# mwhoffman/pygp

Measured on AMD Instinct MI355X. Metric: ExactGP log-lik+grad evals/sec at N=16384 D=8 SE-ARD fp64, higher is better.
Workload: dtype f64; 1 GPU; ExactGP SE-ARD fp64 loglik+grad, N=16384 D=8 (metric config); batched-theta path: 6 independent thetas per GPU per step through gpx_loglik_batch, X/y resident in HBM; safe_mode=False, safe_mode_switches=0, launch=one process, C ABI only (no torch)

## Files before the change

### pygp_amd/csrc/chol.hip

```cpp

#include "gpx_internal.h"

#define LB GPX_TILE

#include <algorithm>
#include <vector>

__global__ __launch_bounds__(256) void copy_block_kernel(const double *__restrict__ src,
                                                         double *__restrict__ dst, int ld,
                                                         int rows, int cols, long long stride)
{
    src += (long long)blockIdx.z * stride;
    dst += (long long)blockIdx.z * stride;
    const int c2 = blockIdx.x * 256 + threadIdx.x;
    if (2 * c2 >= cols) return;
    for (int r = blockIdx.y; r < rows; r += gridDim.y)
        reinterpret_cast<double2 *>(dst + (size_t)r * ld)[c2] =
            reinterpret_cast<const double2 *>(src + (size_t)r * ld)[c2];
}

static int copy_block(hipStream_t s, const double *src, double *dst, int ld, int rows,
                      int cols, int batch = 1, long long stride = 0)
{
    dim3 grid((cols / 2 + 255) / 256, rows < 1024 ? rows : 1024, batch);
// ... 415 lines not shown
    hipEvent_t *G = w.events + 2 * GPX_MAX_BLOCKS;
    hipEvent_t *TD = w.events + 3 * GPX_MAX_BLOCKS;
    bool lead = false;
    if (ahead) {
        GPX_EV(hipEventRecord(D[0], s));
        const bool wide0 = nb > 1 && wide_ok(w, bl.len(0), bl.len(1), 1);
        lead = w.lead && w.lead_rows >= (wide0 ? bl.off(2) : bl.len(0));
        GPX_EV(hipStreamWaitEvent(crit, lead ? w.lead : D[0], 0));
        GPX_EV(hipStreamWaitEvent(bulk, D[0], 0));
        if (aux != bulk) GPX_EV(hipStreamWaitEvent(aux, D[0], 0));
    }
    for (int k = 0; k < nb; ++k) {
        const int ok = bl.off(k), nk = bl.len(k);
        if (ahead && k > 0) GPX_EV(hipStreamWaitEvent(crit, D[k], 0));
        const bool wide = k + 1 < nb && wide_ok(w, nk, bl.len(k + 1), 1);
        if (wide)
            GPX_TRY(gpx_panel(crit, w, ok, nk, bl.len(k + 1), w.gate_total[0], w.gate_total[1]));
        else
            GPX_TRY(potrf_rec(crit, w, ok, nk, true));
        if (ahead) {
            GPX_EV(hipEventRecord(F[k], crit));
            GPX_EV(hipStreamWaitEvent(bulk, F[k], 0));
            if (lead && k == 0) GPX_EV(hipStreamWaitEvent(crit, D[0], 0));
        }
        if (fast && k + 1 < nb) {
            const int o1 = bl.off(k + 1), n1 = bl.len(k + 1), rest = w.np - o1;
            const size_t okk = (size_t)ok * ld + ok, ok1 = (size_t)ok * ld + o1;
            const size_t o11 = (size_t)o1 * ld + o1;
            if (!wide) {
                if (k >= 1) GPX_EV(hipStreamWaitEvent(crit, G[k - 1], 0));
                {
                    GemmArgs g = mk(w.W + okk, ld, w.Kinv + ok1, ld, w.A + ok1, ld, nk, n1, nk,
                                    1.0, 0.0, GEMM_KHI_M);
                    g.order = gpx_env().ord_r12;
                    GPX_TRY(gpx_gemm(crit, 1, 0, g));
                }
                if (k >= 1) GPX_EV(hipStreamWaitEvent(crit, TD[k - 1], 0));
                GPX_TRY(syrk_upper(crit, w.A + ok1, ld, w.A + o11, ld, n1, nk, w.Kinv + o11));
            }
            GPX_EV(hipEventRecord(D[k + 1], crit));
            if (rest > n1) {
                GemmArgs g = mk(w.W + okk, ld, w.Kinv + ok1 + n1, ld, w.A + ok1 + n1, ld, nk,
                                rest - n1, nk, 1.0, 0.0, GEMM_KHI_M);
                g.order = gpx_env().ord_r12;
                GPX_TRY(gpx_gemm(bulk, 1, 0, g));
            }
            GPX_EV(hipStreamWaitEvent(bulk, D[k + 1], 0));
            if (k + 2 < nb) {
                const int o2 = bl.off(k + 2), n2 = bl.len(k + 2), rest2 = w.np - o2;
                const size_t ok2 = (size_t)ok * ld + o2, o12 = (size_t)o1 * ld + o2,
                             o22 = (size_t)o2 * ld + o2;
                {
                    GemmArgs g = mk(w.A + ok1, ld, w.A + ok2, ld, w.Kinv + o12, ld, n1, rest2,
                                    nk, -1.0, 1.0, 0);
                    GPX_TRY(gpx_gemm(bulk, 1, 0, g));
                }
                GPX_TRY(gate_bump(bulk, w, 0));
                GPX_EV(hipEventRecord(G[k], bulk));
                GPX_TRY(syrk_upper(bulk, w.A + ok2, ld, w.A + o22, ld, n2, nk, w.Kinv + o22));
                GPX_TRY(gate_bump(bulk, w, 1));
                GPX_EV(hipEventRecord(TD[k], bulk));
                if (k + 3 < nb) {
                    const int o3 = bl.off(k + 3), rest3 = w.np - o3;
                    const size_t ok3 = (size_t)ok * ld + o3, o23 = (size_t)o2 * ld + o3,
                                 o33 = (size_t)o3 * ld + o3;
                    GemmArgs g = mk(w.A + ok2, ld, w.A + ok3, ld, w.Kinv + o23, ld, n2, rest3, nk,
                                    -1.0, 1.0, 0);
                    GPX_TRY(gpx_gemm(bulk, 1, 0, g));
                    GPX_TRY(syrk_upper(bulk, w.A + ok3, ld, w.A + o33, ld, rest3, nk,
                                       w.Kinv + o33));
                }
            }
        } else if (k + 1 < nb) {
            const int o1 = bl.off(k + 1), n1 = bl.len(k + 1), rest = w.np - o1;
            const size_t okk = (size_t)ok * ld + ok, ok1 = (size_t)ok * ld + o1;
            const int skip = wide ? n1 : 0;
            if (rest > skip) {
                GemmArgs g = mk(w.W + okk, ld, w.Kinv + ok1 + skip, ld, w.A + ok1 + skip, ld, nk,
                                rest - skip, nk, 1.0, 0.0, GEMM_KHI_M);
                g.order = gpx_env().ord_r12;
                GPX_TRY(gpx_gemm(bulk, 1, 0, g));
            }
            const size_t o11 = (size_t)o1 * ld + o1;
            if (!wide)
                GPX_TRY(syrk_upper(bulk, w.A + ok1, ld, w.A + o11, ld, n1, nk, w.Kinv + o11));
            if (ahead) GPX_EV(hipEventRecord(D[k + 1], bulk));
            if (k + 2 < nb) {
                const int o2 = bl.off(k + 2), rest2 = w.np - o2;
                const size_t ok2 = (size_t)ok * ld + o2, o12 = (size_t)o1 * ld + o2,
                             o22 = (size_t)o2 * ld + o2;
                {
                    GemmArgs g = mk(w.A + ok1, ld, w.A + ok2, ld, w.Kinv + o12, ld, n1, rest2,
                                    nk, -1.0, 1.0, 0);
                    GPX_TRY(gpx_gemm(bulk, 1, 0, g));
                }
                GPX_TRY(gate_bump(bulk, w, 0));
                GPX_TRY(syrk_upper(bulk, w.A + ok2, ld, w.A + o22, ld, rest2, nk, w.Kinv + o22));
                GPX_TRY(gate_bump(bulk, w, 1));
            }
        }
        if (mode != GPX_POTRF_R)
            GPX_TRY(inverse_column(aux, w, bl, k, mode == GPX_POTRF_KINV,
                                   defer && k == nb - 1 ? evW : nullptr,
                                   ahead && aux != bulk && k > 0 ? D[k] : nullptr,
                                   ahead && aux != bulk ? F[k] : nullptr));
    }
    if (ahead) {
        GPX_EV(hipEventRecord(evJoin, bulk));
        GPX_EV(hipStreamWaitEvent(s, evJoin, 0));
        if (aux != bulk) {
            GPX_EV(hipEventRecord(evAux, aux));
            GPX_EV(hipStreamWaitEvent(s, defer ? evW : evAux, 0));
        }
    }
    return 0;
}

int gpx_potrf_join(hipStream_t s, const DenseWs &w)
{
    if (w.defer_kinv && w.events && w.aux)
        GPX_EV(hipStreamWaitEvent(s, w.events[4 * GPX_MAX_BLOCKS + 1], 0));
    return 0;
}

hipEvent_t gpx_potrf_lead_event(const DenseWs &w)
{
    return w.events ? w.events[4 * GPX_MAX_BLOCKS + 3] : nullptr;
}

int gpx_trtri(hipStream_t s, const DenseWs &w)
{
    const BatchScope batch_scope(w);
    const Blocks bl(w.np);
    return trtri_blocks(s, w, bl, 0, bl.count);
}

int gpx_trsm_rt(hipStream_t s, const DenseWs &w, double *B, double *T, int ldb, int m,
                long long pstride)
{
    const BatchScope batch_scope(w);
    const Blocks bl(w.np);
    const int ld = w.ld;
    const int nb = w.batch > 1 ? w.batch : 1;
    auto panel = [&](GemmArgs g, bool a_panel) {
        if (nb > 1) {
            if (a_panel) g.strideA = pstride;
            g.strideB = pstride;
            g.strideC = pstride;
        }
        return g;
    };
    for (int k = 0; k < bl.count; ++k) {
        const int ok = bl.off(k), nk = bl.len(k);
        const size_t okk = (size_t)ok * ld + ok;
        double *Bk = B + (size_t)ok * ldb, *Tk = T + (size_t)ok * ldb;
        if (nk == LB) {
            GemmArgs g = mk(w.W + okk, ld, Bk, ldb, Bk, ldb, LB, m, LB, 1.0, 0.0, 0);
            g.tile = 128;
            GPX_TRY(gpx_gemm(s, 1, 0, panel(g, false)));
        } else {
            GPX_TRY(copy_block(s, Bk, Tk, ldb, nk, m, nb, pstride));
            GemmArgs g = mk(w.W + okk, ld, Tk, ldb, Bk, ldb, nk, m, nk, 1.0, 0.0, GEMM_KHI_M);
            g.order = 1;
            GPX_TRY(gpx_gemm(s, 1, 0, panel(g, false)));
        }
        const int o1 = bl.off(k + 1), rest = w.np - o1;
        if (rest > 0)
            GPX_TRY(gpx_gemm(s, 1, 0,
                             panel(mk(w.A + (size_t)ok * ld + o1, ld, Bk, ldb, B + (size_t)o1 * ldb,
                                      ldb, rest, m, nk, -1.0, 1.0, 0), false)));
    }
    return 0;
}

int gpx_lauum(hipStream_t s, const DenseWs &w)
{
    const BatchScope batch_scope(w);
    const int n = w.np, ld = w.ld;
    GemmArgs g = mk(w.W, ld, w.W, ld, w.Kinv, ld, n, n, n, 1.0, 0.0,
                    GEMM_UPPER_ONLY | GEMM_KLO_M | GEMM_KLO_N |
// ... 12 lines not shown
```

### pygp_amd/csrc/gemm_f64.hip

```cpp

#include "gpx_internal.h"

#include "gemm_tile.h"

template <int TA, int TB, typename G>
__global__ __launch_bounds__(G::NTH, G::MINW) void gemm_f64_kernel(GemmArgs g)
{
    constexpr int TILE = G::TILE, WTM = G::WTM, WTN = G::WTN;
    extern __shared__ __attribute__((aligned(16))) char smem_raw[];
    double *smem = reinterpret_cast<double *>(smem_raw);

    int tm = blockIdx.y, tn = blockIdx.x;
    if (g.tiles) {
        tm = g.tiles[2 * blockIdx.x];
        tn = g.tiles[2 * blockIdx.x + 1];
    } else {
        const int gx = gridDim.x, gy = gridDim.y;
        const int mgx = gx >> 3, mgy = gy >> 3;
        const bool macro = g.swizzle && !(gx & 7) && !(gy & 7) && !((mgx * mgy) & 7);
        const int lin = blockIdx.y * gx + blockIdx.x;
        int u = lin, ux = gx, uy = gy;
        int w = 0;
        if (macro) {
            const int xcd = lin & 7, q = lin >> 3;
            u = (q >> 6) * 8 + xcd;
            w = q & 63;
            ux = mgx;
            uy = mgy;
        }
        int um, un;
        if (g.order == 0) {
            um = u / ux; un = u - um * ux;
        } else if (g.order == 1) {
            um = u / ux; un = u - um * ux; um = uy - 1 - um;
        } else {
            un = u / uy; um = u - un * uy;
            if (g.order == 2) un = ux - 1 - un;
        }
        if (macro) {
            tm = um * 8 + (w >> 3);
            tn = un * 8 + (w & 7);
        } else {
            tm = um;
            tn = un;
        }
    }
    const int m0 = tm * TILE, n0 = tn * TILE;
    if ((g.flags & GEMM_UPPER_ONLY) && n0 + TILE <= m0) return;
    int klo = 0, khi = g.K;
    if (g.flags & GEMM_KLO_M) klo = max(klo, m0 - g.kshift);
    if (g.flags & GEMM_KHI_M) khi = min(khi, m0 + TILE);
    if (g.flags & GEMM_KLO_N) klo = max(klo, n0 - g.kshift);
    if (g.flags & GEMM_KHI_N) khi = min(khi, n0 + TILE);
    int zb = blockIdx.z, zm = 0;
    if (g.kchunk > 0) {
        if (g.nsplit > 0) {
            zm = zb / g.nsplit;
            zb -= zm * g.nsplit;
        }
        klo = max(klo, zb * g.kchunk);
        khi = min(khi, (zb + 1) * g.kchunk);
    }
    klo &= ~(BK - 1);

    const double *__restrict__ A = g.A + (long long)zb * g.strideA + (long long)zm * g.mstrideA;
    const double *__restrict__ B = g.B + (long long)zb * g.strideB + (long long)zm * g.mstrideB;
    double *__restrict__ C = g.C + (long long)zb * g.strideC + (long long)zm * g.mstrideC;

    const int tid = threadIdx.x;
    const int lane = tid & 63, wave = tid >> 6;
    const int wm = wave / G::WN, wn = wave % G::WN;
    const int lr = lane & 15, lk = lane >> 4;

    constexpr bool AKM = (TA == 1);
    constexpr bool BKM = (TB == 0);
    constexpr int AK = AKM ? 4 * G::KSTR : 4, AT = AKM ? 16 : 16 * MNSTR;
    constexpr int BKS = BKM ? 4 * G::KSTR : 4, BT = BKM ? 16 : 16 * MNSTR;

    const double alpha = g.alpha;
    const double beta = (g.beta0_from >= 0 && n0 >= g.beta0_from) ? 0.0 : g.beta;
    if (g.C2 && (m0 >> 7) != (n0 >> 7))
        C = g.C2 + (long long)zb * g.strideC2;
    v4d acc[WTM][WTN];
    if (beta != 0.0) {
        const double sc = beta / alpha;
#pragma unroll
        for (int i = 0; i < WTM; ++i)
#pragma unroll
            for (int j = 0; j < WTN; ++j) {
                const int col = n0 + wn * (TILE / G::WN) + j * 16 + lr;
#pragma unroll
                for (int r = 0; r < 4; ++r) {
                    const int row = m0 + wm * (TILE / G::WM) + i * 16 + lk + 4 * r;
                    acc[i][j][r] = sc * C[(size_t)row * g.ldc + col];
                }
            }
    } else {
#pragma unroll
        for (int i = 0; i < WTM; ++i)
#pragma unroll
            for (int j = 0; j < WTN; ++j) acc[i][j] = (v4d){0.0, 0.0, 0.0, 0.0};
    }

    const int nslice = (khi - klo) / BK;
    if (nslice > 0) {
        double *As = smem, *Bs = smem + 2 * G::OPER;
        const bool rev = (g.flags & GEMM_KREV) != 0;
        const int kfirst = rev ? khi - BK : klo, kstep = rev ? -BK : BK;
        const int amn = wm * (TILE / G::WM) + lr, bmn = wn * (TILE / G::WN) + lr;
        const double *ap0 = As + (AKM ? lk * G::KSTR + amn : amn * MNSTR + lk);
        const double *bp0 = Bs + (BKM ? lk * G::KSTR + bmn : bmn * MNSTR + lk);
        if constexpr (!G::DEEP) {
            Regs<G::NLOAD> ra, rb;
            ra = load_slice<G, AKM>(A, g.lda, m0, kfirst, tid);
            rb = load_slice<G, BKM>(B, g.ldb, n0, kfirst, tid);
            store_slice<G, AKM>(As, tid, ra);
            store_slice<G, BKM>(Bs, tid, rb);
            __syncthreads();
            for (int s = 0; s + 1 < nslice; ++s) {
                const int cur = s & 1;
                const int k0 = kfirst + (s + 1) * kstep;
                ra = load_slice<G, AKM>(A, g.lda, m0, k0, tid);
                rb = load_slice<G, BKM>(B, g.ldb, n0, k0, tid);
                mfma_slice<WTM, WTN, AK, AT, BKS, BT>(ap0 + cur * G::OPER,
                                                      bp0 + cur * G::OPER, acc);
                const int nxt = cur ^ 1;
                store_slice<G, AKM>(As + nxt * G::OPER, tid, ra);
                store_slice<G, BKM>(Bs + nxt * G::OPER, tid, rb);
                __syncthreads();
            }
            const int cur = (nslice - 1) & 1;
            mfma_slice<WTM, WTN, AK, AT, BKS, BT>(ap0 + cur * G::OPER, bp0 + cur * G::OPER,
                                                  acc);
        } else {
            Regs<G::NLOAD> ra0, rb0, ra1, rb1;
            const int last = nslice - 1;
            ra0 = load_slice<G, AKM>(A, g.lda, m0, kfirst, tid);
            rb0 = load_slice<G, BKM>(B, g.ldb, n0, kfirst, tid);
            {
                const int k1 = kfirst + min(1, last) * kstep;
                ra1 = load_slice<G, AKM>(A, g.lda, m0, k1, tid);
                rb1 = load_slice<G, BKM>(B, g.ldb, n0, k1, tid);
            }
            store_slice<G, AKM>(As, tid, ra0);
            store_slice<G, BKM>(Bs, tid, rb0);
            __syncthreads();
            for (int s = 0; s < nslice; s += 2) {
                {
                    const int k2 = kfirst + min(s + 2, last) * kstep;
                    ra0 = load_slice<G, AKM>(A, g.lda, m0, k2, tid);
                    rb0 = load_slice<G, BKM>(B, g.ldb, n0, k2, tid);
                    mfma_slice<WTM, WTN, AK, AT, BKS, BT>(ap0, bp0, acc);
                    store_slice<G, AKM>(As + G::OPER, tid, ra1);
                    store_slice<G, BKM>(Bs + G::OPER, tid, rb1);
                    __syncthreads();
                }
                {
                    const int k3 = kfirst + min(s + 3, last) * kstep;
                    ra1 = load_slice<G, AKM>(A, g.lda, m0, k3, tid);
                    rb1 = load_slice<G, BKM>(B, g.ldb, n0, k3, tid);
                    mfma_slice<WTM, WTN, AK, AT, BKS, BT>(ap0 + G::OPER, bp0 + G::OPER, acc);
                    store_slice<G, AKM>(As, tid, ra0);
                    store_slice<G, BKM>(Bs, tid, rb0);
                    __syncthreads();
                }
            }
        }
    }

#pragma unroll
    for (int i = 0; i < WTM; ++i)
#pragma unroll
        for (int j = 0; j < WTN; ++j)
#pragma unroll
            for (int r = 0; r < 4; ++r) {
                const int row = m0 + wm * (TILE / G::WM) + i * 16 + lk + 4 * r;
                const int col = n0 + wn * (TILE / G::WN) + j * 16 + lr;
                C[(size_t)row * g.ldc + col] = alpha * acc[i][j][r];
            }
}

typedef Geo<128, 2, 2> Big4;
typedef Geo<128, 2, 4> Big8;
typedef Geo<64, 2, 2> Small4;
typedef Geo<64, 2, 4> Small8;
typedef Geo<128, 2, 4, true> Big8D;
typedef Geo<64, 2, 4, true> Small8D;

#include <algorithm>
#include <atomic>
#include <cstdio>
#include <cstdlib>
#include <map>
#include <cstring>
#include <mutex>
#include <tuple>
#include <vector>

struct TileList {
    int *dev = nullptr;
    int count = 0;
};

#define GPX_MAX_DEVICES 64
static std::atomic<int> g_concurrent[GPX_MAX_DEVICES];
void gpx_gemm_concurrency(int device, int delta)
{
    if (device >= 0 && device < GPX_MAX_DEVICES) g_concurrent[device] += delta;
}
int gpx_gemm_concurrent(int device)
{
    return device >= 0 && device < GPX_MAX_DEVICES ? g_concurrent[device].load() : 0;
}

static int tile_order(int device)
{
    const int xcd_env = gpx_env().tile_xcd;
    return xcd_env >= 0 ? xcd_env : (gpx_gemm_concurrent(device) > 0 ? 0 : 1);
}

#define GEMM_SLOTS 512

static int tile_list(int device, int xcd_order, int tile, int Tm, int Tn, int K, int flags,
                     TileList *out, int part = 0, int slots = 0, int kshift = 0)
{
    typedef std::tuple<int, int, int, int, int, int, int, int> Key;
    static std::map<Key, TileList> cache;
    static std::mutex mu;
    const int sflags = flags & (GEMM_UPPER_ONLY | GEMM_KLO_M | GEMM_KHI_M | GEMM_KLO_N |
                                GEMM_KHI_N);
    const Key key(device, tile, Tm, Tn, K,
                  sflags | (xcd_order ? 1 << 20 : 0) | ((kshift / 64) << 5), part, slots);
    std::lock_guard<std::mutex> lock(mu);
    auto it = cache.find(key);
    if (it != cache.end()) {
        *out = it->second;
        return 0;
    }
    struct Item { int w, m, n; };
    std::vector<Item> items;
    items.reserve((size_t)Tm * Tn);
    const int gen_tile = part ? 128 : tile;
    for (int m = 0; m < Tm; ++m)
        for (int n = 0; n < Tn; ++n) {
            const int m0 = m * gen_tile, n0 = n * gen_tile;
            if ((sflags & GEMM_UPPER_ONLY) && n0 + gen_tile <= m0) continue;
            int klo = 0, khi = K;
            if (sflags & GEMM_KLO_M) klo = std::max(klo, m0 - kshift);
            if (sflags & GEMM_KHI_M) khi = std::min(khi, m0 + gen_tile);
            if (sflags & GEMM_KLO_N) klo = std::max(klo, n0 - kshift);
            if (sflags & GEMM_KHI_N) khi = std::min(khi, n0 + gen_tile);
            items.push_back({std::max(0, khi - klo), m, n});
// ... 25 lines not shown
                             [](const Item &a, const Item &b) { return a.w > b.w; });
            seq[x].insert(seq[x].end(), t.begin(), t.end());
        }
        std::vector<Item> inter;
        inter.reserve(items.size());
        size_t pos[8] = {0, 0, 0, 0, 0, 0, 0, 0};
        while (inter.size() < items.size()) {
            for (int x = 0; x < 8; ++x) {
                if (pos[x] < seq[x].size()) {
                    inter.push_back(seq[x][pos[x]++]);
                } else {
                    int y = 0;
                    for (int k = 1; k < 8; ++k)
                        if (seq[k].size() - pos[k] > seq[y].size() - pos[y]) y = k;
                    if (pos[y] < seq[y].size()) inter.push_back(seq[y][pos[y]++]);
                }
            }
        }
        items.swap(inter);
    } else {
        std::stable_sort(items.begin(), items.end(),
                         [](const Item &a, const Item &b) { return a.w > b.w; });
    }
    if (part) {
        const size_t whole = slots > 0 ? items.size() / slots * slots : items.size();
        if (part == 1) {
            items.resize(whole);
        } else {
            std::vector<Item> rest;
            for (size_t i = whole; i < items.size(); ++i)
                for (int q = 0; q < 4; ++q) {
                    const int m = 2 * items[i].m + (q >> 1), n = 2 * items[i].n + (q & 1);
                    if ((sflags & GEMM_UPPER_ONLY) && n < m) continue;
                    rest.push_back({items[i].w, m, n});
                }
            items.swap(rest);
        }
    }
    std::vector<int> flat(items.size() * 2);
    for (size_t i = 0; i < items.size(); ++i) {
        flat[2 * i] = items[i].m;
        flat[2 * i + 1] = items[i].n;
    }
    TileList tl;
    tl.count = (int)items.size();
    if (tl.count > 0) {
        GPX_HIP(hipMalloc((void **)&tl.dev, flat.size() * sizeof(int)));
        GPX_HIP(hipMemcpy(tl.dev, flat.data(), flat.size() * sizeof(int),
                          hipMemcpyHostToDevice));
    GPX_HIP(hipDeviceSynchronize());
    }
    cache[key] = tl;
    *out = tl;
    return 0;
}

static void log_launch(hipStream_t s, int ta, int tb, int tile, const GemmArgs &g, int part,
                       int wgs)
{
    static FILE *f = nullptr;
    static bool init = false;
    static std::mutex mu;
    std::lock_guard<std::mutex> lock(mu);
    if (!init) {
        init = true;
        const char *e = gpx_env().gemm_log;
        if (e && *e) f = fopen(e, "w");
    }
    if (!f) return;
    fprintf(f, "%p %d %d %d %d %d %d %d %d %d %d %g\n", (void *)s, ta, tb, tile, g.M, g.N, g.K,
            g.flags, g.kshift, part, wgs, g.beta);
    fflush(f);
}

struct LaunchCtx {
    int device;
    int xcd_order;
};

template <int TA, int TB, typename G>
static int launch(hipStream_t s, const GemmArgs &g0, const LaunchCtx &lc, int part = 0)
{
    GemmArgs g = g0;
    const int structure = g.flags & (GEMM_UPPER_ONLY | GEMM_KLO_M | GEMM_KHI_M |
                                     GEMM_KLO_N | GEMM_KHI_N);
    g.tiles = nullptr;
    dim3 grid(g.N / G::TILE, g.M / G::TILE, g.batch > 0 ? g.batch : 1);
    if (part) {
        TileList tl;
        GPX_TRY(tile_list(lc.device, lc.xcd_order, G::TILE, g.M / 128, g.N / 128, g.K, g.flags,
                          &tl, part, GEMM_SLOTS));
        if (tl.count == 0) return 0;
        g.tiles = tl.dev;
        grid = dim3(tl.count, 1, 1);
    } else if (structure && g.use_lists) {
        TileList tl;
        GPX_TRY(tile_list(lc.device, lc.xcd_order, G::TILE, g.M / G::TILE, g.N / G::TILE, g.K,
                          g.flags, &tl, 0, 0, g.kshift));
        if (tl.count == 0) return 0;
        g.tiles = tl.dev;
        grid = dim3(tl.count, 1, g.batch > 0 ? g.batch : 1);
    }
    log_launch(s, TA, TB, G::TILE, g, part, (int)(grid.x * grid.y * grid.z));
    hipLaunchKernelGGL((gemm_f64_kernel<TA, TB, G>), grid, dim3(G::NTH), G::LDS_BYTES, s,
                       g);
    GPX_HIP(hipGetLastError());
    return 0;
}

template <int TA, int TB, typename G>
static int set_attr()
{
    GPX_HIP(hipFuncSetAttribute(reinterpret_cast<const void *>(&gemm_f64_kernel<TA, TB, G>),
                                hipFuncAttributeMaxDynamicSharedMemorySize, G::LDS_BYTES));
    return 0;
}

template <typename G>
static int set_attr_all()
{
    GPX_TRY((set_attr<0, 0, G>()));
    GPX_TRY((set_attr<0, 1, G>()));
    GPX_TRY((set_attr<1, 0, G>()));
    GPX_TRY((set_attr<1, 1, G>()));
    return 0;
}

int gpx_gemm_init()
{
    GPX_TRY(set_attr_all<Big4>());
    GPX_TRY(set_attr_all<Big8>());
    GPX_TRY(set_attr_all<Small4>());
    GPX_TRY(set_attr_all<Small8>());
    GPX_TRY(set_attr_all<Big8D>());
    GPX_TRY(set_attr_all<Small8D>());
    return 0;
}

template <typename G>
static int dispatch(hipStream_t s, int ta, int tb, const GemmArgs &g, const LaunchCtx &lc,
                    int part = 0)
{
    if (ta == 0 && tb == 0) return launch<0, 0, G>(s, g, lc, part);
    if (ta == 0 && tb == 1) return launch<0, 1, G>(s, g, lc, part);
    if (ta == 1 && tb == 0) return launch<1, 0, G>(s, g, lc, part);
    return launch<1, 1, G>(s, g, lc, part);
}

__global__ void gpx_jitter_kernel(long long ticks)
{
    const long long t0 = wall_clock64();
    while (wall_clock64() - t0 < ticks) __builtin_amdgcn_s_sleep(32);
}

int gpx_test_jitter(hipStream_t s)
{
    if (!gpx_env().test_jitter) return 0;
    static std::mutex mu;
    static unsigned long long state = 0;
    const int max_us = gpx_env().test_jitter_max_us;
    std::lock_guard<std::mutex> lock(mu);
    if (state == 0) state = 0x9E3779B97F4A7C15ull ^ (unsigned long long)gpx_env().test_jitter_seed;
    state = state * 6364136223846793005ull + 1442695040888963407ull;
    const unsigned r = (unsigned)(state >> 33);
    if (r & 1) return 0;
    const long long ticks = (long long)((r >> 1) % (unsigned)(max_us + 1)) * 100;
// ... 90 lines not shown
```

### pygp_amd/csrc/gemm_tile.h

```cpp
#pragma once
#include "gpx_internal.h"

#ifndef GPX_V4D
#define GPX_V4D
typedef double v4d __attribute__((ext_vector_type(4)));
#endif

#define BK GPX_BK
#define MNSTR 18

template <int TILE_, int WM_, int WN_, bool DEEP_ = false> struct Geo {
    static constexpr int TILE = TILE_, WM = WM_, WN = WN_;
    static constexpr bool DEEP = DEEP_;
    static constexpr int NTH = 64 * WM * WN;
    static constexpr int MINW = (WM_ * WN_ >= 8) ? 4 : 2;
    static constexpr int WTM = TILE / WM / 16, WTN = TILE / WN / 16;
    static constexpr int KSTR = TILE + 16;
    static constexpr int OPER = (BK * KSTR > TILE * MNSTR) ? BK * KSTR : TILE * MNSTR;
    static constexpr int LDS_BYTES = 2 * 2 * OPER * 8;
    static constexpr int NLOAD = TILE * BK / 2 / NTH;
    static_assert(NLOAD >= 1 && NLOAD * NTH * 2 == TILE * BK, "loader shape");
};

template <int N> struct Regs { double2 v[N]; };

template <typename G, bool KMAJOR>
__device__ __forceinline__ Regs<G::NLOAD> load_slice(const double *__restrict__ P, int ld,
                                                     int mn0, int k0, int tid)
{
    Regs<G::NLOAD> out;
    double2 (&r)[G::NLOAD] = out.v;
#pragma unroll
    for (int c = 0; c < G::NLOAD; ++c) {
        const int idx = tid + G::NTH * c;
        if (KMAJOR) {
            const int row = idx / (G::TILE / 2), c2 = idx % (G::TILE / 2);
            r[c] = *reinterpret_cast<const double2 *>(P + (size_t)(k0 + row) * ld + mn0 +
                                                      2 * c2);
        } else {
            const int row = idx >> 3, k2 = idx & 7;
            r[c] = *reinterpret_cast<const double2 *>(P + (size_t)(mn0 + row) * ld + k0 +
                                                      2 * k2);
        }
    }
    return out;
}

template <typename G, bool KMAJOR>
__device__ __forceinline__ void store_slice(double *__restrict__ S, int tid,
                                            const Regs<G::NLOAD> &in)
{
    const double2 (&r)[G::NLOAD] = in.v;
#pragma unroll
    for (int c = 0; c < G::NLOAD; ++c) {
        const int idx = tid + G::NTH * c;
        if (KMAJOR) {
            const int row = idx / (G::TILE / 2), c2 = idx % (G::TILE / 2);
            *reinterpret_cast<double2 *>(S + row * G::KSTR + 2 * c2) = r[c];
        } else {
            const int row = idx >> 3, k2 = idx & 7;
            *reinterpret_cast<double2 *>(S + row * MNSTR + 2 * k2) = r[c];
        }
    }
}

template <int WTM, int WTN, int AK, int AT, int BKS, int BT>
__device__ __forceinline__ void mfma_slice(const double *__restrict__ ap,
                                           const double *__restrict__ bp,
                                           v4d (&acc)[WTM][WTN])
{
#pragma unroll
    for (int ks = 0; ks < BK / 4; ++ks) {
        double a[WTM], b[WTN];
#pragma unroll
        for (int t = 0; t < WTM; ++t) a[t] = ap[ks * AK + t * AT];
#pragma unroll
        for (int t = 0; t < WTN; ++t) b[t] = bp[ks * BKS + t * BT];
#pragma unroll
        for (int i = 0; i < WTM; ++i)
#pragma unroll
            for (int j = 0; j < WTN; ++j)
                acc[i][j] = __builtin_amdgcn_mfma_f64_16x16x4f64(a[i], b[j], acc[i][j],
                                                                 0, 0, 0);
    }
}
```

### pygp_amd/csrc/gpx_env.h

```cpp
#pragma once

#include <cstdlib>
#include <cstring>
#include <vector>

#define GPX_ENV_TABLE(X)                                                        \
        \
    X(int, nb0, "GPX_NB0", 0)                                                   \
    X(int, nb, "GPX_NB", 0)                                                     \
    X(const char *, blocks_text, "GPX_BLOCKS", nullptr)                         \
    X(int, split_last, "GPX_SPLIT_LAST", 0)                                     \
    X(int, lookahead, "GPX_LOOKAHEAD", 1)                                       \
    X(int, fastchain, "GPX_FASTCHAIN", 1)                                       \
    X(int, aux, "GPX_AUX", 1)                                                   \
    X(int, lead_build, "GPX_LEAD_BUILD", 1)                                     \
    X(int, defer_kinv, "GPX_DEFER_KINV", 1)                                     \
    X(int, invcol_early, "GPX_INVCOL_EARLY", -1)                                \
    X(int, overlap_nosplit, "GPX_OVERLAP_NOSPLIT", 1)                           \
    X(int, grad_whole, "GPX_GRAD_WHOLE", 4096)                                  \
    X(int, grad_full_w, "GPX_GRAD_FULL_W", 4096)                                \
       \
    X(int, swizzle, "GPX_SWIZZLE", 0)                                           \
    X(int, tile_lists, "GPX_TILE_LISTS", 1)                                     \
    X(int, ord_t, "GPX_ORD_T", 2)                                               \
    X(int, ord_r12, "GPX_ORD_R12", 1)                                           \
    X(int, ord_lauum, "GPX_ORD_LAUUM", 0)                                       \
    X(int, krev, "GPX_KREV", 0)                                                 \
    X(int, krev_invcol, "GPX_KREV_INVCOL", 0)                                   \
    X(int, tile_xcd, "GPX_TILE_XCD", -1)                                        \
    X(int, gemm_big, "GPX_GEMM_BIG", 0)                                         \
    X(int, gemm_small, "GPX_GEMM_SMALL", 0)                                     \
    X(int, gemm_small_below, "GPX_GEMM_SMALL_BELOW", 0)                         \
    X(int, gemm_nobalance, "GPX_GEMM_NOBALANCE", 0)                             \
    X(int, gemm_nosplit, "GPX_GEMM_NOSPLIT", 0)                                 \
    X(const char *, gemm_log, "GPX_GEMM_LOG", nullptr)                          \
    X(int, ldpad, "GPX_LDPAD", 32)                                              \
    X(int, bench_ldpad, "GPX_BENCH_LDPAD", 0)                                   \
                                           \
    X(int, panel, "GPX_PANEL", -1)                                              \
    X(int, panel_stream, "GPX_PANEL_STREAM", 1)                                 \
    X(int, panel_serial, "GPX_PANEL_SERIAL", 1)                                 \
    X(int, panel_strict, "GPX_PANEL_STRICT", 0)                                 \
    X(int, panel_debug, "GPX_PANEL_DEBUG", 0)                                   \
    X(int, panel_timeout_ms, "GPX_PANEL_TIMEOUT_MS", 2000)                      \
    X(int, panel_timeout_us, "GPX_PANEL_TIMEOUT_US", 0)                         \
    X(int, panel_wg, "GPX_PANEL_WG", -1)                                        \
    X(int, panel_wg_wide, "GPX_PANEL_WG_WIDE", -1)                              \
    X(int, panel_wg_whole, "GPX_PANEL_WG_WHOLE", -1)                            \
    X(int, panel_nspine, "GPX_PANEL_NSPINE", -1)                                \
    X(int, panel_mspine, "GPX_PANEL_MSPINE", -1)                                \
    X(int, panel_mwg, "GPX_PANEL_MWG", -1)                                      \
    X(int, panel_split, "GPX_PANEL_SPLIT", 1)                                   \
    X(int, panel_fold, "GPX_PANEL_FOLD", 1)                                     \
    X(int, panel_kbatch, "GPX_PANEL_KBATCH", -1)                                \
    X(int, panel_i128, "GPX_PANEL_I128", -1)                                    \
    X(int, panel_u128, "GPX_PANEL_U128", 6)                                     \
    X(double, panel_chain_scale, "GPX_PANEL_CHAIN_SCALE", 0.75)                 \
    X(int, panel_whole, "GPX_PANEL_WHOLE", GPX_PANEL_WHOLE_DEFAULT)             \
    X(int, panel_rhs, "GPX_PANEL_RHS", 1)                                       \
    X(int, panel_wide, "GPX_PANEL_WIDE", 0)                                     \
    X(int, panel_leaf_skip, "GPX_PANEL_LEAF_SKIP", 0)                           \
    X(int, leaf_skip, "GPX_LEAF_SKIP", 0)                                       \
    X(int, leaf_mfma, "GPX_LEAF_MFMA", 1)                                       \
     \
    X(int, group_max_np, "GPX_GROUP_MAX_NP", 32768)                             \
    X(int, group_members, "GPX_GROUP_MEMBERS", 0)                               \
    X(int, group_inflight, "GPX_GROUP_INFLIGHT", 0)                             \
    X(int, group_min_big, "GPX_GROUP_MIN_BIG", 2)                               \
    X(int, sweep_min_members, "GPX_SWEEP_MIN_MEMBERS", 16)                      \
    X(int, sweep_lite, "GPX_SWEEP_LITE", 1)                                     \
    X(int, sweep_fold, "GPX_SWEEP_FOLD", -1)                                    \
    X(int, sweep_pre, "GPX_SWEEP_PRE", 1)                                       \
    X(int, sweep_right, "GPX_SWEEP_RIGHT", 4)                                   \
    X(int, sweep_invblock, "GPX_SWEEP_INVBLOCK", 4)                             \
    X(int, sweep_narrow, "GPX_SWEEP_NARROW", 1)                                 \
    X(int, sweep_rhs_dense, "GPX_SWEEP_RHS_DENSE", 1)                           \
    X(int, solo_max_np, "GPX_SOLO_MAX_NP", 0)                                   \
    X(int, solo_min_members, "GPX_SOLO_MIN_MEMBERS", 16)                        \
    X(int, xs_debug, "GPX_XS_DEBUG", 0)                                         \
     \
    X(int, batch_inflight, "GPX_BATCH_INFLIGHT", 3)                             \
    X(int, batch_lookahead, "GPX_BATCH_LOOKAHEAD", -1)                          \
    X(int, twin_probe, "GPX_TWIN_PROBE", 1)                                     \
    X(int, twin_own_bulk, "GPX_TWIN_OWN_BULK", 1)                               \
    X(bool, twin_log, "GPX_TWIN_LOG", false)                                    \
    X(bool, destroy_log, "GPX_DESTROY_LOG", false)                              \
    X(int, multi_fake, "GPX_MULTI_FAKE", 0)                                     \
    X(int, multi_force_rccl, "GPX_MULTI_FORCE_RCCL", 0)                         \
                                          \
    X(int, kbuild_w, "GPX_KBUILD_W", 0)                                         \
    X(int, trace_rows, "GPX_TRACE_ROWS", 16)                                    \
                                                                \
    X(const char *, test_jitter_text, "GPX_TEST_JITTER", nullptr)               \
    X(int, test_hold_build_us, "GPX_TEST_HOLD_BUILD_US", 0)

struct GpxEnv {
#define GPX_ENV_FIELD(type, field, name, dflt) type field;
    GPX_ENV_TABLE(GPX_ENV_FIELD)
#undef GPX_ENV_FIELD
    std::vector<int> blocks;
    bool test_jitter;
    long long test_jitter_seed;
    int test_jitter_max_us;

    static int read(const char *e, int dflt) { return e ? atoi(e) : dflt; }
    static double read(const char *e, double dflt) { return e ? atof(e) : dflt; }
// ... 48 lines not shown
```

### pygp_amd/csrc/gpx_internal.h

```cpp
#pragma once

#include <hip/hip_runtime.h>
#include <math.h>
#include <stdint.h>
#include <string>
#include <vector>

#include "../../include/gpx.h"

#define GPX_TILE 128
#define GPX_BK 16
#define GPX_PANEL_MAX 1024
#define GPX_PANEL_WHOLE_MAX 4096
#define GPX_PANEL_WHOLE_DEFAULT 4096
#define PANEL_IG 8

#include "gpx_env.h"

void gpx_set_error(const char *fmt, ...);
#define GPX_HIP(expr)                                                          \
    do {                                                                       \
        hipError_t e_ = (expr);                                                \
        if (e_ != hipSuccess) {                                                \
            gpx_set_error("%s:%d: %s -> %s", __FILE__, __LINE__, #expr,        \
// ... 20 lines not shown
    {
        if (need <= bytes) return 0;
        if (p) GPX_HIP(hipFree(p));
        p = nullptr;
        bytes = 0;
        GPX_HIP(hipMalloc(&p, need));
        bytes = need;
        return 0;
    }
    void release()
    {
        if (p) (void)hipFree(p);
        p = nullptr;
        bytes = 0;
    }
    template <typename T> T *as() const { return static_cast<T *>(p); }
    double *d() const { return as<double>(); }
};

struct KPart {
    int kind;
    int iso;
    int nhyper;
    int hoff;
    int group;
    int dup;
    double two_logsf;
    double sf2;
    double ell;
    double pi_over_p;
    double period;
    double alpha;
    double scale[GPX_MAX_DIM];
};
struct KParams {
    int nparts;
    int ndim;
    int nhyper;
    int nprod;
    KPart part[GPX_MAX_PARTS];
};
int gpx_flatten_kspec(const gpx_kspec *k, int64_t d, KParams *out);

struct MemberParams {
    KParams kp;
    double sn2;
    double mean;
    double prior;
    double pad_;
};
struct MemberBatch {
    int count = 1;
    const MemberParams *params = nullptr;
    long long mstride = 0;
    long long vstride = 0;
};
int gpx_kspec_with_hyper(const gpx_kspec *k, const double *hyper,
                         std::vector<gpx_kspec> &store, gpx_kspec *out);

enum {
    GEMM_UPPER_ONLY = 1,
    GEMM_KLO_M = 2,
    GEMM_KHI_M = 4,
    GEMM_KLO_N = 8,
    GEMM_KHI_N = 16,
    GEMM_KREV = 32,
};
struct GemmArgs {
    const double *A = nullptr;
    const double *B = nullptr;
    double *C = nullptr;
    int lda = 0, ldb = 0, ldc = 0;
    int M = 0, N = 0, K = 0;
    double alpha = 1.0, beta = 0.0;
    long long strideA = 0, strideB = 0, strideC = 0;
    int batch = 1;
    int flags = 0;
    int tile = 0;
    int order = 0;
    int swizzle = 0;
    int waves = 0;
    int use_lists = 1;
    const int *tiles = nullptr;
    double *C2 = nullptr;
    int kshift = 0;
    int beta0_from = -1;
    int overlap = 0;
    long long strideC2 = 0;
    int kchunk = 0;
    int nsplit = 0;
    long long mstrideA = 0, mstrideB = 0, mstrideC = 0;
};
int gpx_gemm(hipStream_t s, int ta, int tb, const GemmArgs &g);
void gpx_gemm_concurrency(int device, int delta);
int gpx_gemm_concurrent(int device);


struct DenseWs {
    double *A = nullptr;
    double *W = nullptr;
    double *Kinv = nullptr;
    int np = 0;
    int ld = 0;
    int *info = nullptr;
    int *pctl = nullptr;
    int batch = 1;
    long long mstride = 0;
    int pstride = 0;
    bool whole = false;
    bool no_inverse = false;
    bool full_w = false;
    int *gate_total = nullptr;
    hipStream_t crit = nullptr, aux = nullptr, bulk = nullptr;
    hipEvent_t *events = nullptr;
    hipEvent_t lead = nullptr;
    int lead_rows = 0;
    bool defer_kinv = false;
    bool aug_rhs = false;
};
#define GPX_MAX_BLOCKS 64
#define GPX_LA_EVENTS (4 * GPX_MAX_BLOCKS + 4)
int gpx_block_layout(int np, int *offs, bool full_inverse = false);
struct GpxBlocks {
    int np, count;
    int offs[GPX_MAX_BLOCKS + 1];
    explicit GpxBlocks(int np_, bool full_inverse = false) : np(np_)
    {
        count = gpx_block_layout(np, offs, full_inverse);
    }
    int off(int k) const { return k <= 0 ? 0 : (k >= count ? np : offs[k]); }
    int len(int k) const { return off(k + 1) - off(k); }
};
enum { GPX_POTRF_R = 0, GPX_POTRF_W = 1, GPX_POTRF_KINV = 2 };
int gpx_potrf(hipStream_t s, const DenseWs &w, int mode, bool offdiag_staged);
bool gpx_potrf_whole(const DenseWs &w, int mode);
int gpx_grad_mode(const DenseWs &w);
bool gpx_grad_full_w(const DenseWs &w, int mode);
bool gpx_potrf_rhs_ok(const DenseWs &w, int mode);
int gpx_test_jitter(hipStream_t s);
int gpx_potrf_join(hipStream_t s, const DenseWs &w);
hipEvent_t gpx_potrf_lead_event(const DenseWs &w);
int gpx_trtri(hipStream_t s, const DenseWs &w);
int gpx_lauum(hipStream_t s, const DenseWs &w);
int gpx_aat_upper(hipStream_t s, const DenseWs &w, const double *S, double *C);
int gpx_trsm_rt(hipStream_t s, const DenseWs &w, double *B, double *T, int ldb, int m,
                long long pstride = 0);

size_t gpx_trsv_scratch(int np);
int gpx_trsv_rt(hipStream_t s, const DenseWs &w, bool w_complete, double *r_scratch,
                double *a, double *partial, long long vstride = 0);
int gpx_rt_residual(hipStream_t s, const double *R, int ld, int np, const double *V,
                    double *B, int ldb, int m, int batch = 1, long long mstride = 0,
                    long long pstride = 0);
int gpx_add_inplace(hipStream_t s, double *x, const double *d, size_t n);
int gpx_trmv_upper(hipStream_t s, const double *W, int ld, int np, const double *v,
                   double *out, int batch = 1, long long mstride = 0, long long vstride = 0);
int gpx_lz_terms(hipStream_t s, const double *R, int ld, int n, const double *a,
                 const double *alpha, double *scalars, int batch = 1, long long mstride = 0,
                 long long vstride = 0, int sstride = 0, const int *info = nullptr,
                 int astride = 1);
int gpx_residual(hipStream_t s, const double *y, double mean, int n, int np,
                 double *r);
int gpx_residual_members(hipStream_t s, const double *y, const MemberBatch &mb, int n, int np,
                         double *r, double *aug, int ld, int *info_zero = nullptr);
int gpx_residual_rhs(hipStream_t s, const double *y, double mean, int n, int np, double *r,
                     double *aug, int ld);
// ... 217 lines not shown
```

Baseline: 14.65 evals/s.

## Skip structurally-zero MFMA blocks in f64 GEMM and merge trailing SYRK updates

Adds a ZeroSkip mask in the f64 GEMM kernel. K-slices that touch known-zero triangular regions (KLO/KHI/UPPER_ONLY flags) are run through a masked MFMA path that skips dead 16x16 sub-tiles, and waves whose diagonal-tile output is entirely unneeded skip the C load and store. Separately, when look-ahead is off, the Cholesky trailing update replaces the SYRK+GEMM+SYRK sequence with one larger SYRK over the remaining columns, which cuts launch count. The masked path adds branching and code size in the inner loop. The merged SYRK may do somewhat more or less work depending on how it handles the off-diagonal block.

Result: no change. 14.72 evals/s (median of 6 runs) (+0.5%).

```diff
diff --git a/pygp_amd/csrc/chol.hip b/pygp_amd/csrc/chol.hip
--- a/pygp_amd/csrc/chol.hip
+++ b/pygp_amd/csrc/chol.hip
@@ -521,20 +521,26 @@
                 GPX_TRY(gpx_gemm(bulk, 1, 0, g));
             }
             const size_t o11 = (size_t)o1 * ld + o1;
-            if (!wide)
-                GPX_TRY(syrk_upper(bulk, w.A + ok1, ld, w.A + o11, ld, n1, nk, w.Kinv + o11));
-            if (ahead) GPX_EV(hipEventRecord(D[k + 1], bulk));
+            const bool merged = !ahead && !wide && gpx_env().trailing_merge;
+            if (merged) {
+                GPX_TRY(syrk_upper(bulk, w.A + ok1, ld, w.A + o11, ld, rest, nk, w.Kinv + o11));
+            } else {
+                if (!wide)
+                    GPX_TRY(syrk_upper(bulk, w.A + ok1, ld, w.A + o11, ld, n1, nk, w.Kinv + o11));
+                if (ahead) GPX_EV(hipEventRecord(D[k + 1], bulk));
+            }
             if (k + 2 < nb) {
                 const int o2 = bl.off(k + 2), rest2 = w.np - o2;
                 const size_t ok2 = (size_t)ok * ld + o2, o12 = (size_t)o1 * ld + o2,
                              o22 = (size_t)o2 * ld + o2;
-                {
+                if (!merged) {
                     GemmArgs g = mk(w.A + ok1, ld, w.A + ok2, ld, w.Kinv + o12, ld, n1, rest2,
                                     nk, -1.0, 1.0, 0);
                     GPX_TRY(gpx_gemm(bulk, 1, 0, g));
                 }
                 GPX_TRY(gate_bump(bulk, w, 0));
-                GPX_TRY(syrk_upper(bulk, w.A + ok2, ld, w.A + o22, ld, rest2, nk, w.Kinv + o22));
+                if (!merged)
+                    GPX_TRY(syrk_upper(bulk, w.A + ok2, ld, w.A + o22, ld, rest2, nk, w.Kinv + o22));
                 GPX_TRY(gate_bump(bulk, w, 1));
             }
         }
diff --git a/pygp_amd/csrc/gemm_f64.hip b/pygp_amd/csrc/gemm_f64.hip
--- a/pygp_amd/csrc/gemm_f64.hip
+++ b/pygp_amd/csrc/gemm_f64.hip
@@ -2,6 +2,8 @@
 #include "gpx_internal.h"
 
 #include "gemm_tile.h"
+
+#include <type_traits>
 
 template <int TA, int TB, typename G>
 __global__ __launch_bounds__(G::NTH, G::MINW) void gemm_f64_kernel(GemmArgs g)
@@ -81,8 +83,28 @@
     const double beta = (g.beta0_from >= 0 && n0 >= g.beta0_from) ? 0.0 : g.beta;
     if (g.C2 && (m0 >> 7) != (n0 >> 7))
         C = g.C2 + (long long)zb * g.strideC2;
+    ZeroSkip zs;
+    int wg_lo = klo, wg_hi = khi;
+    {
+        const int uw = __builtin_amdgcn_readfirstlane(wave);
+        const int uwm = uw / G::WN, uwn = uw % G::WN;
+        zs.mfirst = m0 + uwm * (TILE / G::WM);
+        zs.nfirst = n0 + uwn * (TILE / G::WN);
+        zs.flags = g.zero_skip ? g.flags : 0;
+        zs.kshift = g.kshift;
+        zs.none = false;
+        if (zs.flags & GEMM_KLO_M) wg_lo = max(wg_lo, m0 + TILE - 16 - g.kshift);
+        if (zs.flags & GEMM_KLO_N) wg_lo = max(wg_lo, n0 + TILE - 16 - g.kshift);
+        if (zs.flags & GEMM_KHI_M) wg_hi = min(wg_hi, m0 + 15);
+        if (zs.flags & GEMM_KHI_N) wg_hi = min(wg_hi, n0 + 15);
+        if (TILE == 128 && (zs.flags & GEMM_UPPER_ONLY) && m0 == n0) {
+            wg_hi = klo - 1;
+            zs.none = uwm * (TILE / G::WM) >= 64 && (uwn + 1) * (TILE / G::WN) <= 64;
+        }
+    }
+    const bool none = __builtin_amdgcn_readfirstlane((int)zs.none);
     v4d acc[WTM][WTN];
-    if (beta != 0.0) {
+    if (beta != 0.0 && !none) {
         const double sc = beta / alpha;
 #pragma unroll
         for (int i = 0; i < WTM; ++i)
@@ -110,6 +132,16 @@
         const int amn = wm * (TILE / G::WM) + lr, bmn = wn * (TILE / G::WN) + lr;
         const double *ap0 = As + (AKM ? lk * G::KSTR + amn : amn * MNSTR + lk);
         const double *bp0 = Bs + (BKM ? lk * G::KSTR + bmn : bmn * MNSTR + lk);
+        int sA, sB;
+        {
+            const int d = wg_lo - klo, e = wg_hi - klo;
+            const int tA = d <= 0 ? 0 : min(nslice, (d + BK - 1) / BK);
+            const int tB = e < 0 ? tA : max(tA, min(nslice, e / BK + 1));
+            sA = rev ? nslice - tB : tA;
+            sB = rev ? nslice - tA : tB;
+        }
+        const std::true_type masked;
+        const std::false_type plain;
         if constexpr (!G::DEEP) {
             Regs<G::NLOAD> ra, rb;
             ra = load_slice<G, AKM>(A, g.lda, m0, kfirst, tid);
@@ -117,21 +149,29 @@
             store_slice<G, AKM>(As, tid, ra);
             store_slice<G, BKM>(Bs, tid, rb);
             __syncthreads();
-            for (int s = 0; s + 1 < nslice; ++s) {
-                const int cur = s & 1;
-                const int k0 = kfirst + (s + 1) * kstep;
-                ra = load_slice<G, AKM>(A, g.lda, m0, k0, tid);
-                rb = load_slice<G, BKM>(B, g.ldb, n0, k0, tid);
-                mfma_slice<WTM, WTN, AK, AT, BKS, BT>(ap0 + cur * G::OPER,
-                                                      bp0 + cur * G::OPER, acc);
-                const int nxt = cur ^ 1;
-                store_slice<G, AKM>(As + nxt * G::OPER, tid, ra);
-                store_slice<G, BKM>(Bs + nxt * G::OPER, tid, rb);
-                __syncthreads();
+            auto walk = [&](auto mode, int s0, int s1) {
+                for (int s = s0; s < s1; ++s) {
+                    const int cur = s & 1;
+                    const int k0 = kfirst + (s + 1) * kstep;
+                    ra = load_slice<G, AKM>(A, g.lda, m0, k0, tid);
+                    rb = load_slice<G, BKM>(B, g.ldb, n0, k0, tid);
+                    mfma_slice_at<decltype(mode)::value, WTM, WTN, AK, AT, BKS, BT>(
+                        ap0 + cur * G::OPER, bp0 + cur * G::OPER, acc, k0 - kstep, zs);
+                    const int nxt = cur ^ 1;
+                    store_slice<G, AKM>(As + nxt * G::OPER, tid, ra);
+                    store_slice<G, BKM>(Bs + nxt * G::OPER, tid, rb);
+                    __syncthreads();
+                }
+            };
+            const int body = nslice - 1;
+#pragma unroll 1
+            for (int round = 0; round < 2; ++round) {
+                walk(masked, round ? sB : 0, round ? body : min(sA, body));
+                walk(plain, round ? body : sA, round ? body : min(sB, body));
             }
             const int cur = (nslice - 1) & 1;
-            mfma_slice<WTM, WTN, AK, AT, BKS, BT>(ap0 + cur * G::OPER, bp0 + cur * G::OPER,
-                                                  acc);
+            mfma_slice_at<true, WTM, WTN, AK, AT, BKS, BT>(
+                ap0 + cur * G::OPER, bp0 + cur * G::OPER, acc, kfirst + (nslice - 1) * kstep, zs);
         } else {
             Regs<G::NLOAD> ra0, rb0, ra1, rb1;
             const int last = nslice - 1;
@@ -145,29 +185,40 @@
             store_slice<G, AKM>(As, tid, ra0);
             store_slice<G, BKM>(Bs, tid, rb0);
             __syncthreads();
-            for (int s = 0; s < nslice; s += 2) {
-                {
-                    const int k2 = kfirst + min(s + 2, last) * kstep;
-                    ra0 = load_slice<G, AKM>(A, g.lda, m0, k2, tid);
-                    rb0 = load_slice<G, BKM>(B, g.ldb, n0, k2, tid);
-                    mfma_slice<WTM, WTN, AK, AT, BKS, BT>(ap0, bp0, acc);
-                    store_slice<G, AKM>(As + G::OPER, tid, ra1);
-                    store_slice<G, BKM>(Bs + G::OPER, tid, rb1);
-                    __syncthreads();
+            auto walk = [&](auto mode, int s0, int s1) {
+                for (int s = s0; s < s1; s += 2) {
+                    {
+                        const int k2 = kfirst + min(s + 2, last) * kstep;
+                        ra0 = load_slice<G, AKM>(A, g.lda, m0, k2, tid);
+                        rb0 = load_slice<G, BKM>(B, g.ldb, n0, k2, tid);
+                        mfma_slice_at<decltype(mode)::value, WTM, WTN, AK, AT, BKS, BT>(
+                            ap0, bp0, acc, kfirst + s * kstep, zs);
+                        store_slice<G, AKM>(As + G::OPER, tid, ra1);
+                        store_slice<G, BKM>(Bs + G::OPER, tid, rb1);
+                        __syncthreads();
+                    }
+                    {
+                        const int k3 = kfirst + min(s + 3, last) * kstep;
+                        ra1 = load_slice<G, AKM>(A, g.lda, m0, k3, tid);
+                        rb1 = load_slice<G, BKM>(B, g.ldb, n0, k3, tid);
+                        mfma_slice_at<decltype(mode)::value, WTM, WTN, AK, AT, BKS, BT>(
+                            ap0 + G::OPER, bp0 + G::OPER, acc, kfirst + (s + 1) * kstep, zs);
+                        store_slice<G, AKM>(As, tid, ra0);
+                        store_slice<G, BKM>(Bs, tid, rb0);
+                        __syncthreads();
+                    }
                 }
-                {
-                    const int k3 = kfirst + min(s + 3, last) * kstep;
-                    ra1 = load_slice<G, AKM>(A, g.lda, m0, k3, tid);
-                    rb1 = load_slice<G, BKM>(B, g.ldb, n0, k3, tid);
-                    mfma_slice<WTM, WTN, AK, AT, BKS, BT>(ap0 + G::OPER, bp0 + G::OPER, acc);
-                    store_slice<G, AKM>(As, tid, ra0);
-                    store_slice<G, BKM>(Bs, tid, rb0);
-                    __syncthreads();
-                }
-            }
-        }
-    }
-
+            };
+            const int pA = (sA + 1) & ~1, pB = max(pA, sB & ~1);
+#pragma unroll 1
+            for (int round = 0; round < 2; ++round) {
+                walk(masked, round ? pB : 0, round ? nslice : pA);
+                walk(plain, round ? nslice : pA, round ? nslice : pB);
+            }
+        }
+    }
+
+    if (none) return;
 #pragma unroll
     for (int i = 0; i < WTM; ++i)
 #pragma unroll
@@ -359,6 +410,7 @@
 static int launch(hipStream_t s, const GemmArgs &g0, const LaunchCtx &lc, int part = 0)
 {
     GemmArgs g = g0;
+    g.zero_skip = gpx_env().zero_skip;
     const int structure = g.flags & (GEMM_UPPER_ONLY | GEMM_KLO_M | GEMM_KHI_M |
                                      GEMM_KLO_N | GEMM_KHI_N);
     g.tiles = nullptr;
diff --git a/pygp_amd/csrc/gemm_tile.h b/pygp_amd/csrc/gemm_tile.h
--- a/pygp_amd/csrc/gemm_tile.h
+++ b/pygp_amd/csrc/gemm_tile.h
@@ -84,3 +84,70 @@
                                                                  0, 0, 0);
     }
 }
+
+struct ZeroSkip {
+    int mfirst, nfirst;
+    int flags, kshift;
+    bool none;
+
+    template <int WT>
+    __device__ __forceinline__ unsigned live(int k, int first, bool lo, bool hi) const
+    {
+        unsigned m = 0;
+#pragma unroll
+        for (int t = 0; t < WT; ++t) {
+            const int f = first + 16 * t;
+            const bool dead = (lo && k + 15 < f - kshift) || (hi && k > f + 15);
+            m |= (dead ? 0u : 1u) << t;
+        }
+        return none ? 0u : m;
+    }
+    template <int WTM> __device__ __forceinline__ unsigned rows(int k) const
+    {
+        return live<WTM>(k, mfirst, flags & GEMM_KLO_M, flags & GEMM_KHI_M);
+    }
+    template <int WTN> __device__ __forceinline__ unsigned cols(int k) const
+    {
+        return live<WTN>(k, nfirst, flags & GEMM_KLO_N, flags & GEMM_KHI_N);
+    }
+};
+
+template <int WTM, int WTN, int AK, int AT, int BKS, int BT>
+__device__ __forceinline__ void mfma_slice_masked(const double *__restrict__ ap,
+                                                  const double *__restrict__ bp,
+                                                  v4d (&acc)[WTM][WTN], unsigned rm, unsigned cm)
+{
+#pragma unroll
+    for (int ks = 0; ks < BK / 4; ++ks) {
+        double a[WTM], b[WTN];
+#pragma unroll
+        for (int t = 0; t < WTM; ++t) a[t] = ap[ks * AK + t * AT];
+#pragma unroll
+        for (int t = 0; t < WTN; ++t) b[t] = bp[ks * BKS + t * BT];
+#pragma unroll
+        for (int i = 0; i < WTM; ++i)
+            if (rm >> i & 1) {
+#pragma unroll
+                for (int j = 0; j < WTN; ++j)
+                    if (cm >> j & 1) {
+                        asm volatile("");
+                        acc[i][j] = __builtin_amdgcn_mfma_f64_16x16x4f64(a[i], b[j], acc[i][j],
+                                                                         0, 0, 0);
+                    }
+            }
+    }
+}
+
+template <bool MASKED, int WTM, int WTN, int AK, int AT, int BKS, int BT>
+__device__ __forceinline__ void mfma_slice_at(const double *__restrict__ ap,
+                                              const double *__restrict__ bp,
+                                              v4d (&acc)[WTM][WTN], int k, const ZeroSkip &z)
+{
+    if constexpr (!MASKED) {
+        mfma_slice<WTM, WTN, AK, AT, BKS, BT>(ap, bp, acc);
+    } else {
+        const unsigned rm = __builtin_amdgcn_readfirstlane(z.rows<WTM>(k));
+        const unsigned cm = __builtin_amdgcn_readfirstlane(z.cols<WTN>(k));
+        mfma_slice_masked<WTM, WTN, AK, AT, BKS, BT>(ap, bp, acc, rm, cm);
+    }
+}
diff --git a/pygp_amd/csrc/gpx_env.h b/pygp_amd/csrc/gpx_env.h
--- a/pygp_amd/csrc/gpx_env.h
+++ b/pygp_amd/csrc/gpx_env.h
@@ -15,6 +15,7 @@
     X(int, aux, "GPX_AUX", 1)                                                   \
     X(int, lead_build, "GPX_LEAD_BUILD", 1)                                     \
     X(int, defer_kinv, "GPX_DEFER_KINV", 1)                                     \
+    X(int, trailing_merge, "GPX_TRAILING_MERGE", 1)                             \
     X(int, invcol_early, "GPX_INVCOL_EARLY", -1)                                \
     X(int, overlap_nosplit, "GPX_OVERLAP_NOSPLIT", 1)                           \
     X(int, grad_whole, "GPX_GRAD_WHOLE", 4096)                                  \
@@ -22,6 +23,7 @@
        \
     X(int, swizzle, "GPX_SWIZZLE", 0)                                           \
     X(int, tile_lists, "GPX_TILE_LISTS", 1)                                     \
+    X(int, zero_skip, "GPX_ZERO_SKIP", 1)                                       \
     X(int, ord_t, "GPX_ORD_T", 2)                                               \
     X(int, ord_r12, "GPX_ORD_R12", 1)                                           \
     X(int, ord_lauum, "GPX_ORD_LAUUM", 0)                                       \
diff --git a/pygp_amd/csrc/gpx_internal.h b/pygp_amd/csrc/gpx_internal.h
--- a/pygp_amd/csrc/gpx_internal.h
+++ b/pygp_amd/csrc/gpx_internal.h
@@ -126,6 +126,7 @@
     int waves = 0;
     int use_lists = 1;
     const int *tiles = nullptr;
+    int zero_skip = 0;
     double *C2 = nullptr;
     int kshift = 0;
     int beta0_from = -1;
```
